# Nyro-Robotics/booster_gym

Measured on AMD Instinct MI355X. Metric: env-steps/sec (whole node), PPO rollout+update, T1 4096 envs/GPU, higher is better.
Workload: dtype f32

## Files before the change

booster_gym_amd/csrc/bg_wgrad_split.hip:

```cpp
#include <hip/hip_runtime.h>

#include <type_traits>

#include "bg_wgrad.h"

#define BG_MFMA(ACC, A, B) ACC = __builtin_amdgcn_mfma_f32_32x32x16_bf16(__builtin_bit_cast(bf16x8, A), __builtin_bit_cast(bf16x8, B), ACC, 0, 0, 0)
#define BG_PIN() __builtin_amdgcn_sched_barrier(0)

constexpr int WS_BLOCK = 16;
constexpr int WS_LDS_FLOATS = 36864;
__device__ float ws_zero_block[WS_BLOCK * 512];

struct Pair3 { unsigned h, m, l; };
__device__ __forceinline__ Pair3 split_pair3(float x0, float x1) {
    const unsigned u0 = __float_as_uint(x0), u1 = __float_as_uint(x1);
    Pair3 o;
    o.h = __builtin_amdgcn_perm(u1, u0, 0x07060302u);
    const float r0 = x0 - __uint_as_float(u0 & 0xffff0000u), r1 = x1 - __uint_as_float(u1 & 0xffff0000u);
    const unsigned v0 = __float_as_uint(r0), v1 = __float_as_uint(r1);
    o.m = __builtin_amdgcn_perm(v1, v0, 0x07060302u);
    const float s0 = r0 - __uint_as_float(v0 & 0xffff0000u), s1 = r1 - __uint_as_float(v1 & 0xffff0000u);
    o.l = __builtin_amdgcn_perm(__float_as_uint(s1), __float_as_uint(s0), 0x07060302u);
    return o;
}
__device__ __forceinline__ void set_dword(u32x4 (&pl)[3], int p, const Pair3& v) {
    pl[0][p] = v.h; pl[1][p] = v.m; pl[2][p] = v.l;
}

struct SplitUnit { unsigned u0, u1, t0, t1; float r0, r1; };
template <int NU>
__device__ __forceinline__ void split_op(int o, SplitUnit (&s)[4], const float (&x)[4], const float (&y)[4], Pair3 (&out)[4], int NG, unsigned sgn) {
    const int k = o % NU;
    SplitUnit& q = s[k];
    switch (o / NU) {
        case 0: {
            const unsigned f = k < NG ? sgn : 0u;
            q.u0 = __float_as_uint(x[k]) ^ f; q.u1 = __float_as_uint(y[k]) ^ f; out[k].h = __builtin_amdgcn_perm(q.u1, q.u0, 0x07060302u);
        } break;
        case 1: q.t0 = q.u0 & 0xffff0000u; break;
        case 2: q.t1 = q.u1 & 0xffff0000u; break;
        case 3: q.r0 = __uint_as_float(q.u0) - __uint_as_float(q.t0); break;
        case 4: q.r1 = __uint_as_float(q.u1) - __uint_as_float(q.t1); break;
        case 5: out[k].m = __builtin_amdgcn_perm(__float_as_uint(q.r1), __float_as_uint(q.r0), 0x07060302u); break;
        case 6: q.t0 = __float_as_uint(q.r0) & 0xffff0000u; break;
        case 7: q.t1 = __float_as_uint(q.r1) & 0xffff0000u; break;
        case 8: q.r0 = q.r0 - __uint_as_float(q.t0); break;
        case 9: q.r1 = q.r1 - __uint_as_float(q.t1); break;
        default: out[k].l = __builtin_amdgcn_perm(__float_as_uint(q.r1), __float_as_uint(q.r0), 0x07060302u); break;
    }
}
template <int TERMS, int NU>
__device__ __forceinline__ void tile_mfmas(f32x16& acc, const u32x4 (&g)[3], const u32x4 (&a)[3], const float (&x)[4], const float (&y)[4], Pair3 (&o)[4], unsigned sgn) {
    constexpr int GP[9] = {2, 1, 2, 0, 1, 2, 0, 1, 0}, AP[9] = {2, 2, 1, 2, 1, 0, 1, 0, 0};
    constexpr int NOPS = 11 * NU;
    SplitUnit s[4];
#pragma unroll
    for (int m = 0; m < TERMS; m++) {
        const int term = 9 - TERMS + m;
        BG_MFMA(acc, g[GP[term]], a[AP[term]]);
#pragma unroll
        for (int op = (m * NOPS) / TERMS; op < ((m + 1) * NOPS) / TERMS; op++) {
            split_op<NU == 0 ? 1 : NU>(op, s, x, y, o, NU - 1, sgn);
        }
        BG_PIN();
    }
}

template <int Cout, int Cin, int TERMS>
__device__ __forceinline__ void wgrad_split_tile(float* lds, int M, const float* __restrict__ G, const float* __restrict__ A,
                                                 float* __restrict__ P, int ntile_ci, int tile0, int tw, int slice, int slices) {
    constexpr int TCI = Cin == 64 ? 2 : 4;
    constexpr int UPG = 4 / TCI;
    typedef float avec __attribute__((ext_vector_type(TCI)));
    const int wave = __builtin_amdgcn_readfirstlane(threadIdx.x >> 6), lane = threadIdx.x & 63, i = lane & 31, h = lane >> 5;
    const int ks = 4 / tw, tl = wave % tw, ksub = wave / tw, tile = tile0 + tl;
    const int tco = tile / ntile_ci, tci = tile % ntile_ci;
    const long NB2 = M / (2 * WS_BLOCK), W = (long)slices * ks, widx = (long)slice * ks + ksub;
    const int b0 = 2 * (int)(NB2 * widx / W), b1 = 2 * (int)(NB2 * (widx + 1) / W), nb = b1 - b0;
    const unsigned sgn = (widx & 1) ? 0x80000000u : 0u;
    auto sg = [&](float v) { return __uint_as_float(__float_as_uint(v) ^ sgn); };
    constexpr int gfl = WS_BLOCK * Cout, afl = WS_BLOCK * Cin, grp_fl = gfl + afl;
    const int buf_fl = ks * grp_fl;
    float* my0 = lds + ksub * grp_fl;
    constexpr int NT = (Cout / 128) * (Cin >= 128 ? Cin / 128 : 1), KS = 4 / NT, NBUF = 3 * KS * grp_fl <= WS_LDS_FLOATS ? 3 : 2;
    constexpr int n_inst = grp_fl / 256, N_MINE = n_inst / NT;
    static_assert(n_inst % NT == 0, "every wave of a group issues the same number of copies");
    auto stage = [&](int blk) {
        const bool real = blk < nb;
        const float* gsrc = real ? G + (size_t)(b0 + blk) * gfl : ws_zero_block;
        const float* asrc = real ? A + (size_t)(b0 + blk) * afl : ws_zero_block;
        float* dst = my0 + (blk % NBUF) * buf_fl;
#pragma unroll
        for (int j = 0; j < N_MINE; j++) {
            const int f = (tl + j * NT) * 256;
            const float* src = f < gfl ? gsrc + f : asrc + (f - gfl);
            __builtin_amdgcn_global_load_lds((const __attribute__((address_space(1))) void*)(src + lane * 4), (__attribute__((address_space(3))) void*)(dst + f), 16, 0, 0);
        }
    };
    const int gofs = (8 * h) * Cout + tco * 128 + 4 * i, aofs = gfl + (8 * h) * Cin + tci * (32 * TCI) + TCI * i;

    f32x16 acc[4][TCI];
#pragma unroll
    for (int t = 0; t < 4; t++)
#pragma unroll
        for (int u = 0; u < TCI; u++)
#pragma unroll
            for (int r = 0; r < 16; r++) acc[t][u][r] = 0.f;
    u32x4 gp[2][4][3], ap[2][TCI][3];

#pragma unroll
    for (int c = 0; c < NBUF; c++) stage(c);
    __builtin_amdgcn_s_waitcnt(0x0F70 | ((NBUF - 1) * N_MINE & 15) | (((NBUF - 1) * N_MINE >> 4) << 14));
    __builtin_amdgcn_s_barrier();
    {
        const float* src = my0;
#pragma unroll
        for (int p = 0; p < 4; p++) {
#pragma unroll
            for (int t = 0; t < 4; t++) set_dword(gp[0][t], p, split_pair3(sg(src[gofs + (2 * p) * Cout + t]), sg(src[gofs + (2 * p + 1) * Cout + t])));
#pragma unroll
            for (int u = 0; u < TCI; u++) set_dword(ap[0][u], p, split_pair3(src[aofs + (2 * p) * Cin + u], src[aofs + (2 * p + 1) * Cin + u]));
        }
    }
    auto block = [&](auto cur_c, const float* src) {
        constexpr int CUR = decltype(cur_c)::value, NXT = 1 - CUR;
        f32x4 gq[2][2]; avec aq[2][2];
        auto rd = [&](int t, int w) {
            gq[w][0] = *reinterpret_cast<const f32x4*>(src + gofs + (2 * t) * Cout); gq[w][1] = *reinterpret_cast<const f32x4*>(src + gofs + (2 * t + 1) * Cout);
            aq[w][0] = *reinterpret_cast<const avec*>(src + aofs + (2 * t) * Cin); aq[w][1] = *reinterpret_cast<const avec*>(src + aofs + (2 * t + 1) * Cin);
        };
        rd(0, 0);
#pragma unroll
        for (int t = 0; t < 4; t++) {
            if (t < 3) rd(t + 1, (t + 1) & 1);
            BG_PIN();
            const f32x4 g0 = gq[t & 1][0], g1 = gq[t & 1][1];
            const avec a0 = aq[t & 1][0], a1 = aq[t & 1][1];
#pragma unroll
            for (int u = 0; u < TCI; u++) {
                float x[4], y[4];
                Pair3 o[4];
#pragma unroll
                for (int k = 0; k < UPG; k++) { x[k] = g0[u * UPG + k]; y[k] = g1[u * UPG + k]; }
                x[UPG] = a0[u]; y[UPG] = a1[u];
                BG_PIN();
                tile_mfmas<TERMS, UPG + 1>(acc[t][u], gp[CUR][t], ap[CUR][u], x, y, o, sgn);
#pragma unroll
                for (int k = 0; k < UPG; k++) set_dword(gp[NXT][u * UPG + k], t, o[k]);
                set_dword(ap[NXT][u], t, o[UPG]);
            }
        }
    };
    using c0 = std::integral_constant<int, 0>; using c1 = std::integral_constant<int, 1>;
    auto top = [&](int c) {
        __builtin_amdgcn_s_waitcnt(0x0F70 | ((NBUF - 2) * N_MINE & 15) | (((NBUF - 2) * N_MINE >> 4) << 14));
        __builtin_amdgcn_s_barrier();
        stage(c + NBUF);
    };
    int nbmax = 0;
    for (int c = 0; c < ks; c++) {
        const long wc = (long)slice * ks + c;
        const int len = 2 * (int)(NB2 * (wc + 1) / W) - 2 * (int)(NB2 * wc / W);
        nbmax = len > nbmax ? len : nbmax;
    }
    for (int b = 0; b < nbmax; b += 2) {
        top(b);
        block(c0{}, my0 + ((b + 1) % NBUF) * buf_fl);
        top(b + 1);
        block(c1{}, my0 + ((b + 2) % NBUF) * buf_fl);
    }
    __builtin_amdgcn_s_waitcnt(0x0F70);
    __syncthreads();
    float (*red)[64 * 16 * 2 * TCI] = reinterpret_cast<float (*)[64 * 16 * 2 * TCI]>(lds);
    float* pt = P + (size_t)slice * Cout * Cin + (size_t)(tco * 128) * Cin + tci * (32 * TCI) + TCI * i;
    const int ipw = 32 / ks;
#pragma unroll
    for (int half = 0; half < 2; half++) {
        if (half) __syncthreads();
#pragma unroll
        for (int tt = 0; tt < 2; tt++)
#pragma unroll
            for (int r = 0; r < 16; r++) {
                avec v;
#pragma unroll
                for (int u = 0; u < TCI; u++) v[u] = acc[2 * half + tt][u][r];
                *reinterpret_cast<avec*>(&red[wave][((tt * 16 + r) * 64 + lane) * TCI]) = v;
            }
        __syncthreads();
        for (int k = 0; k < ipw; k++) {
            const int it = ksub * ipw + k, tt = it >> 4, r = it & 15, idx = ((tt * 16 + r) * 64 + lane) * TCI;
            avec v = *reinterpret_cast<const avec*>(&red[tl][idx]);
            if (((long)slice * ks) & 1) v = -v;
            for (int c = 1; c < ks; c++) {
                const avec w = *reinterpret_cast<const avec*>(&red[tl + tw * c][idx]);
                if (((long)slice * ks + c) & 1) v -= w; else v += w;
            }
            const int row = (r & 3) + 8 * (r >> 2) + 4 * h, t = 2 * half + tt;
            *reinterpret_cast<avec*>(pt + (size_t)(4 * row + t) * Cin) = v;
        }
    }
}

template <int TERMS>
__global__ __launch_bounds__(256, 1) void mlp_wgrad_group_split_kernel(WgradGroup grp) {
    __shared__ __attribute__((aligned(16))) float lds[WS_LDS_FLOATS];
    const int b = blockIdx.x;
    int k = 0;
#pragma unroll
    for (int j = 1; j < WG_MAX_PROBLEMS; j++)
        if (j < grp.np && b >= grp.p[j].wg_begin) k = j;
    const WgradProblem& pr = grp.p[k];
    const int groups = pr.ntiles / pr.tw, local = b - pr.wg_begin, tile0 = (local % groups) * pr.tw, slice = local / groups;
    if (pr.Cout == 256 && pr.Cin == 256) wgrad_split_tile<256, 256, TERMS>(lds, pr.M, pr.G, pr.A, pr.P, pr.ntile_ci, tile0, pr.tw, slice, pr.slices);
    else if (pr.Cout == 128 && pr.Cin == 256) wgrad_split_tile<128, 256, TERMS>(lds, pr.M, pr.G, pr.A, pr.P, pr.ntile_ci, tile0, pr.tw, slice, pr.slices);
    else if (pr.Cout == 128 && pr.Cin == 128) wgrad_split_tile<128, 128, TERMS>(lds, pr.M, pr.G, pr.A, pr.P, pr.ntile_ci, tile0, pr.tw, slice, pr.slices);
    else wgrad_split_tile<256, 64, TERMS>(lds, pr.M, pr.G, pr.A, pr.P, pr.ntile_ci, tile0, pr.tw, slice, pr.slices);
}

static int split_launch(const bg_wgrad_problem* problems, int32_t count, int32_t terms, void* stream, bool finish) {
    if (terms != 9 && terms != 6) return bg_set_error(-4, "bg_mlp_weight_grad_group_split: terms must be 9 or 6");
    WgradGroup grp;
    int wg = 0, fin = 0;
    const int rc = bg_wgrad_group_fill(problems, count, grp, wg, fin, "bg_mlp_weight_grad_group_split");
    if (rc) return rc;
    for (int k = 0; k < count; k++) {
        const WgradProblem& p = grp.p[k];
        if (p.tw != p.ntiles) return bg_set_error(-4, "bg_mlp_weight_grad_group_split: tiles_per_workgroup must equal the layer's tile count (1, 2 or 4)");
        if (p.M % (2 * WS_BLOCK) != 0) return bg_set_error(-4, "bg_mlp_weight_grad_group_split: M must be a multiple of 32");
        if ((long)p.slices * (4 / p.tw) > p.M / (2 * WS_BLOCK)) return bg_set_error(-4, "bg_mlp_weight_grad_group_split: too many slices for M");
        if ((4 / p.tw) * WS_BLOCK * (p.Cout + p.Cin) * 2 > WS_LDS_FLOATS) return bg_set_error(-4, "bg_mlp_weight_grad_group_split: layer too wide for the LDS staging");
        const bool known = (p.Cout == 256 && (p.Cin == 256 || p.Cin == 64)) || (p.Cout == 128 && (p.Cin == 256 || p.Cin == 128));
        if (!known) return bg_set_error(-4, "bg_mlp_weight_grad_group_split: unsupported shape (256 x 256, 128 x 256, 128 x 128, 256 x 64)");
    }
    hipStream_t st = (hipStream_t)stream;
    if (terms == 9) hipLaunchKernelGGL(mlp_wgrad_group_split_kernel<9>, dim3(wg), dim3(256), 0, st, grp);
    else hipLaunchKernelGGL(mlp_wgrad_group_split_kernel<6>, dim3(wg), dim3(256), 0, st, grp);
    if (finish && bg_wgrad_group_finish_launch(grp, fin, st)) return bg_set_error(-2, "bg_mlp_weight_grad_group_split: launch failed");
    HIP_OK(hipGetLastError());
    return 0;
}

extern "C" int bg_mlp_weight_grad_group_split(const bg_wgrad_problem* problems, int32_t count, int32_t terms, void* stream) {
    return split_launch(problems, count, terms, stream, true);
}
extern "C" int bg_mlp_weight_grad_group_split_partial(const bg_wgrad_problem* problems, int32_t count, int32_t terms, void* stream) {
    return split_launch(problems, count, terms, stream, false);
}
```

Measured before the change: 4.582 million.

## Split each wgrad tile across two half-waves groups with 512-thread workgroups

Doubles the workgroup to 512 threads so that each tile's four 32-row MFMA subtiles are split between two wave halves, each holding half the accumulators. The bf16 three-way split pipeline is reworked to keep raw values and split them one block ahead without the double-buffered CUR/NXT register sets. Each block is now processed per iteration instead of two per iteration. The change also adds timestamp probe instrumentation. It aims to lower register pressure and raise MFMA issue parallelism per CU, at the cost of more complex per-wave bookkeeping and extra reduction synchronisation.

```diff
diff --git a/booster_gym_amd/csrc/bg_wgrad_split.hip b/booster_gym_amd/csrc/bg_wgrad_split.hip
--- a/booster_gym_amd/csrc/bg_wgrad_split.hip
+++ b/booster_gym_amd/csrc/bg_wgrad_split.hip
@@ -2,7 +2,10 @@
 
 #include <type_traits>
 
+#include "bg_stamps.h"
 #include "bg_wgrad.h"
+
+BG_STAMP_BUFFER(ws_stamps, bg_probe_read_wgrad_split_stamps, 512, 4)
 
 #define BG_MFMA(ACC, A, B) ACC = __builtin_amdgcn_mfma_f32_32x32x16_bf16(__builtin_bit_cast(bf16x8, A), __builtin_bit_cast(bf16x8, B), ACC, 0, 0, 0)
 #define BG_PIN() __builtin_amdgcn_sched_barrier(0)
@@ -50,7 +53,7 @@
     }
 }
 template <int TERMS, int NU>
-__device__ __forceinline__ void tile_mfmas(f32x16& acc, const u32x4 (&g)[3], const u32x4 (&a)[3], const float (&x)[4], const float (&y)[4], Pair3 (&o)[4], unsigned sgn) {
+__device__ __forceinline__ void tile_mfmas(f32x16& acc, const u32x4 (&g)[3], const u32x4 (&a)[3], const float (&x)[4], const float (&y)[4], Pair3 (&o)[4], int ng, unsigned sgn) {
     constexpr int GP[9] = {2, 1, 2, 0, 1, 2, 0, 1, 0}, AP[9] = {2, 2, 1, 2, 1, 0, 1, 0, 0};
     constexpr int NOPS = 11 * NU;
     SplitUnit s[4];
@@ -60,7 +63,7 @@
         BG_MFMA(acc, g[GP[term]], a[AP[term]]);
 #pragma unroll
         for (int op = (m * NOPS) / TERMS; op < ((m + 1) * NOPS) / TERMS; op++) {
-            split_op<NU == 0 ? 1 : NU>(op, s, x, y, o, NU - 1, sgn);
+            split_op<NU == 0 ? 1 : NU>(op, s, x, y, o, ng, sgn);
         }
         BG_PIN();
     }
@@ -70,9 +73,10 @@
 __device__ __forceinline__ void wgrad_split_tile(float* lds, int M, const float* __restrict__ G, const float* __restrict__ A,
                                                  float* __restrict__ P, int ntile_ci, int tile0, int tw, int slice, int slices) {
     constexpr int TCI = Cin == 64 ? 2 : 4;
-    constexpr int UPG = 4 / TCI;
     typedef float avec __attribute__((ext_vector_type(TCI)));
-    const int wave = __builtin_amdgcn_readfirstlane(threadIdx.x >> 6), lane = threadIdx.x & 63, i = lane & 31, h = lane >> 5;
+    typedef float f32x2 __attribute__((ext_vector_type(2)));
+    const int wave8 = __builtin_amdgcn_readfirstlane(threadIdx.x >> 6), wave = wave8 & 3, hf = wave8 >> 2;
+    const int lane = threadIdx.x & 63, i = lane & 31, h = lane >> 5;
     const int ks = 4 / tw, tl = wave % tw, ksub = wave / tw, tile = tile0 + tl;
     const int tco = tile / ntile_ci, tci = tile % ntile_ci;
     const long NB2 = M / (2 * WS_BLOCK), W = (long)slices * ks, widx = (long)slice * ks + ksub;
@@ -83,8 +87,9 @@
     const int buf_fl = ks * grp_fl;
     float* my0 = lds + ksub * grp_fl;
     constexpr int NT = (Cout / 128) * (Cin >= 128 ? Cin / 128 : 1), KS = 4 / NT, NBUF = 3 * KS * grp_fl <= WS_LDS_FLOATS ? 3 : 2;
-    constexpr int n_inst = grp_fl / 256, N_MINE = n_inst / NT;
-    static_assert(n_inst % NT == 0, "every wave of a group issues the same number of copies");
+    constexpr int n_inst = grp_fl / 256, N_MINE = n_inst / (2 * NT);
+    static_assert(n_inst % (2 * NT) == 0, "every wave of a group issues the same number of copies");
+    static_assert((NBUF - 1) * N_MINE < 64, "the counted waits below have six bits");
     auto stage = [&](int blk) {
         const bool real = blk < nb;
         const float* gsrc = real ? G + (size_t)(b0 + blk) * gfl : ws_zero_block;
@@ -92,21 +97,22 @@
         float* dst = my0 + (blk % NBUF) * buf_fl;
 #pragma unroll
         for (int j = 0; j < N_MINE; j++) {
-            const int f = (tl + j * NT) * 256;
+            const int f = (2 * tl + hf + j * 2 * NT) * 256;
             const float* src = f < gfl ? gsrc + f : asrc + (f - gfl);
             __builtin_amdgcn_global_load_lds((const __attribute__((address_space(1))) void*)(src + lane * 4), (__attribute__((address_space(3))) void*)(dst + f), 16, 0, 0);
         }
     };
-    const int gofs = (8 * h) * Cout + tco * 128 + 4 * i, aofs = gfl + (8 * h) * Cin + tci * (32 * TCI) + TCI * i;
-
-    f32x16 acc[4][TCI];
-#pragma unroll
-    for (int t = 0; t < 4; t++)
+    const int gofs = (8 * h) * Cout + tco * 128 + 4 * i + 2 * hf, aofs = gfl + (8 * h) * Cin + tci * (32 * TCI) + TCI * i;
+
+    f32x16 acc[2][TCI];
+#pragma unroll
+    for (int t = 0; t < 2; t++)
 #pragma unroll
         for (int u = 0; u < TCI; u++)
 #pragma unroll
             for (int r = 0; r < 16; r++) acc[t][u][r] = 0.f;
-    u32x4 gp[2][4][3], ap[2][TCI][3];
+    u32x4 gp[2][3], ap[TCI][3];
+    float rawG[8], rawA[8];
 
 #pragma unroll
     for (int c = 0; c < NBUF; c++) stage(c);
@@ -116,79 +122,104 @@
         const float* src = my0;
 #pragma unroll
         for (int p = 0; p < 4; p++) {
-#pragma unroll
-            for (int t = 0; t < 4; t++) set_dword(gp[0][t], p, split_pair3(sg(src[gofs + (2 * p) * Cout + t]), sg(src[gofs + (2 * p + 1) * Cout + t])));
-#pragma unroll
-            for (int u = 0; u < TCI; u++) set_dword(ap[0][u], p, split_pair3(src[aofs + (2 * p) * Cin + u], src[aofs + (2 * p + 1) * Cin + u]));
-        }
-    }
-    auto block = [&](auto cur_c, const float* src) {
-        constexpr int CUR = decltype(cur_c)::value, NXT = 1 - CUR;
-        f32x4 gq[2][2]; avec aq[2][2];
-        auto rd = [&](int t, int w) {
-            gq[w][0] = *reinterpret_cast<const f32x4*>(src + gofs + (2 * t) * Cout); gq[w][1] = *reinterpret_cast<const f32x4*>(src + gofs + (2 * t + 1) * Cout);
-            aq[w][0] = *reinterpret_cast<const avec*>(src + aofs + (2 * t) * Cin); aq[w][1] = *reinterpret_cast<const avec*>(src + aofs + (2 * t + 1) * Cin);
-        };
-        rd(0, 0);
-#pragma unroll
-        for (int t = 0; t < 4; t++) {
-            if (t < 3) rd(t + 1, (t + 1) & 1);
+            set_dword(gp[0], p, split_pair3(sg(src[gofs + (2 * p) * Cout]), sg(src[gofs + (2 * p + 1) * Cout])));
+#pragma unroll
+            for (int u = 0; u < TCI - 1; u++) set_dword(ap[u], p, split_pair3(src[aofs + (2 * p) * Cin + u], src[aofs + (2 * p + 1) * Cin + u]));
+        }
+#pragma unroll
+        for (int r = 0; r < 8; r++) { rawG[r] = src[gofs + r * Cout + 1]; rawA[r] = src[aofs + r * Cin + TCI - 1]; }
+    }
+    auto block = [&](const float* src) {
+        float hold[8];
+#pragma unroll
+        for (int u = 0; u < TCI; u++) {
+            constexpr int UP0 = 8 / TCI;
+            float x[4], y[4];
+            Pair3 o[4];
+#pragma unroll
+            for (int k = 0; k < UP0; k++) {
+                const int f = u * UP0 + k, p = f & 3;
+                x[k] = f < 4 ? rawA[2 * p] : rawG[2 * p]; y[k] = f < 4 ? rawA[2 * p + 1] : rawG[2 * p + 1];
+            }
             BG_PIN();
-            const f32x4 g0 = gq[t & 1][0], g1 = gq[t & 1][1];
-            const avec a0 = aq[t & 1][0], a1 = aq[t & 1][1];
-#pragma unroll
-            for (int u = 0; u < TCI; u++) {
-                float x[4], y[4];
-                Pair3 o[4];
-#pragma unroll
-                for (int k = 0; k < UPG; k++) { x[k] = g0[u * UPG + k]; y[k] = g1[u * UPG + k]; }
-                x[UPG] = a0[u]; y[UPG] = a1[u];
-                BG_PIN();
-                tile_mfmas<TERMS, UPG + 1>(acc[t][u], gp[CUR][t], ap[CUR][u], x, y, o, sgn);
-#pragma unroll
-                for (int k = 0; k < UPG; k++) set_dword(gp[NXT][u * UPG + k], t, o[k]);
-                set_dword(ap[NXT][u], t, o[UPG]);
+            tile_mfmas<TERMS, UP0>(acc[0][u], gp[0], ap[u], x, y, o, u * UP0 >= 4 ? UP0 : 0, sgn);
+#pragma unroll
+            for (int k = 0; k < UP0; k++) {
+                const int f = u * UP0 + k, p = f & 3;
+                if (f < 4) set_dword(ap[TCI - 1], p, o[k]); else set_dword(gp[1], p, o[k]);
+            }
+        }
+#pragma unroll
+        for (int u = 0; u < TCI; u++) {
+            float x[4], y[4];
+            Pair3 o[4];
+            if (u == 0) {
+#pragma unroll
+                for (int r = 0; r < 8; r++) {
+                    const f32x2 v = *reinterpret_cast<const f32x2*>(src + gofs + r * Cout);
+                    if (r & 1) y[r >> 1] = v[0]; else x[r >> 1] = v[0];
+                    rawG[r] = v[1];
+                }
+            } else if (u & 1) {
+#pragma unroll
+                for (int r = 0; r < 8; r++) {
+                    const f32x2 v = *reinterpret_cast<const f32x2*>(src + aofs + r * Cin + (u - 1));
+                    if (r & 1) y[r >> 1] = v[0]; else x[r >> 1] = v[0];
+                    if (u == TCI - 1) rawA[r] = v[1]; else hold[r] = v[1];
+                }
+            } else {
+#pragma unroll
+                for (int k = 0; k < 4; k++) { x[k] = hold[2 * k]; y[k] = hold[2 * k + 1]; }
+            }
+            BG_PIN();
+            tile_mfmas<TERMS, 4>(acc[1][u], gp[1], ap[u], x, y, o, u == 0 ? 4 : 0, sgn);
+#pragma unroll
+            for (int k = 0; k < 4; k++) {
+                if (u == 0) set_dword(gp[0], k, o[k]); else set_dword(ap[u > 0 ? u - 1 : 0], k, o[k]);
             }
         }
     };
-    using c0 = std::integral_constant<int, 0>; using c1 = std::integral_constant<int, 1>;
     auto top = [&](int c) {
         __builtin_amdgcn_s_waitcnt(0x0F70 | ((NBUF - 2) * N_MINE & 15) | (((NBUF - 2) * N_MINE >> 4) << 14));
         __builtin_amdgcn_s_barrier();
         stage(c + NBUF);
     };
+    BG_STAMP_LOCALS(4);
     int nbmax = 0;
     for (int c = 0; c < ks; c++) {
         const long wc = (long)slice * ks + c;
         const int len = 2 * (int)(NB2 * (wc + 1) / W) - 2 * (int)(NB2 * wc / W);
         nbmax = len > nbmax ? len : nbmax;
     }
-    for (int b = 0; b < nbmax; b += 2) {
+    BG_STAMP_FENCED(0); BG_STAMP_WALL(2);
+    for (int b = 0; b < nbmax; b++) {
         top(b);
-        block(c0{}, my0 + ((b + 1) % NBUF) * buf_fl);
-        top(b + 1);
-        block(c1{}, my0 + ((b + 2) % NBUF) * buf_fl);
-    }
+        block(my0 + ((b + 1) % NBUF) * buf_fl);
+    }
+    BG_STAMP_FENCED(1); BG_STAMP_WALL(3);
+    BG_STAMP_FLUSH(ws_stamps, 4, blockIdx.x < 256, 2 * blockIdx.x);
     __builtin_amdgcn_s_waitcnt(0x0F70);
     __syncthreads();
     float (*red)[64 * 16 * 2 * TCI] = reinterpret_cast<float (*)[64 * 16 * 2 * TCI]>(lds);
     float* pt = P + (size_t)slice * Cout * Cin + (size_t)(tco * 128) * Cin + tci * (32 * TCI) + TCI * i;
-    const int ipw = 32 / ks;
+    const int ipw = 16 / ks;
 #pragma unroll
     for (int half = 0; half < 2; half++) {
         if (half) __syncthreads();
-#pragma unroll
-        for (int tt = 0; tt < 2; tt++)
-#pragma unroll
-            for (int r = 0; r < 16; r++) {
-                avec v;
-#pragma unroll
-                for (int u = 0; u < TCI; u++) v[u] = acc[2 * half + tt][u][r];
-                *reinterpret_cast<avec*>(&red[wave][((tt * 16 + r) * 64 + lane) * TCI]) = v;
-            }
+        if (hf == half) {
+#pragma unroll
+            for (int tt = 0; tt < 2; tt++)
+#pragma unroll
+                for (int r = 0; r < 16; r++) {
+                    avec v;
+#pragma unroll
+                    for (int u = 0; u < TCI; u++) v[u] = acc[tt][u][r];
+                    *reinterpret_cast<avec*>(&red[wave][((tt * 16 + r) * 64 + lane) * TCI]) = v;
+                }
+        }
         __syncthreads();
         for (int k = 0; k < ipw; k++) {
-            const int it = ksub * ipw + k, tt = it >> 4, r = it & 15, idx = ((tt * 16 + r) * 64 + lane) * TCI;
+            const int it = (2 * ksub + hf) * ipw + k, tt = it >> 4, r = it & 15, idx = ((tt * 16 + r) * 64 + lane) * TCI;
             avec v = *reinterpret_cast<const avec*>(&red[tl][idx]);
             if (((long)slice * ks) & 1) v = -v;
             for (int c = 1; c < ks; c++) {
@@ -202,7 +233,7 @@
 }
 
 template <int TERMS>
-__global__ __launch_bounds__(256, 1) void mlp_wgrad_group_split_kernel(WgradGroup grp) {
+__global__ __launch_bounds__(512, 1) void mlp_wgrad_group_split_kernel(WgradGroup grp) {
     __shared__ __attribute__((aligned(16))) float lds[WS_LDS_FLOATS];
     const int b = blockIdx.x;
     int k = 0;
@@ -233,8 +264,8 @@
         if (!known) return bg_set_error(-4, "bg_mlp_weight_grad_group_split: unsupported shape (256 x 256, 128 x 256, 128 x 128, 256 x 64)");
     }
     hipStream_t st = (hipStream_t)stream;
-    if (terms == 9) hipLaunchKernelGGL(mlp_wgrad_group_split_kernel<9>, dim3(wg), dim3(256), 0, st, grp);
-    else hipLaunchKernelGGL(mlp_wgrad_group_split_kernel<6>, dim3(wg), dim3(256), 0, st, grp);
+    if (terms == 9) hipLaunchKernelGGL(mlp_wgrad_group_split_kernel<9>, dim3(wg), dim3(512), 0, st, grp);
+    else hipLaunchKernelGGL(mlp_wgrad_group_split_kernel<6>, dim3(wg), dim3(512), 0, st, grp);
     if (finish && bg_wgrad_group_finish_launch(grp, fin, st)) return bg_set_error(-2, "bg_mlp_weight_grad_group_split: launch failed");
     HIP_OK(hipGetLastError());
     return 0;
```

After: 4.558 million. About the same (-0.5%).
